# diff7/tts-king

Hardware: AMD Instinct MI355X
Metric: FS2 train mel-frames/sec/GPU + HiFi-GAN RTF (22.05 kHz), batch=16 (higher is better)
Workload: dtype bf16

## Files before the change

### include/ttsk.h

```cpp
#ifndef TTSK_H
#define TTSK_H

#include <stdint.h>

#ifdef __cplusplus
extern "C" {
#endif

#define TTSK_VERSION 1

#define TTSK_OK 0
#define TTSK_EINVAL (-1)
#define TTSK_ELAUNCH (-2)

int ttsk_version(void);
const char* ttsk_last_error(void);

enum {
  TTSK_GEMM_A_TR      = 1 << 0,
  TTSK_GEMM_B_TR      = 1 << 1,
  TTSK_GEMM_C_F32     = 1 << 2,
  TTSK_GEMM_RELU      = 1 << 3,
  TTSK_GEMM_ADD_R     = 1 << 4,
  TTSK_GEMM_R_F32     = 1 << 5,
  TTSK_GEMM_MASK_G    = 1 << 6,
  TTSK_GEMM_LRELU_IN  = 1 << 7,
  TTSK_GEMM_TANH      = 1 << 8,
  TTSK_GEMM_ACCUM_C   = 1 << 9,
  TTSK_GEMM_LRELU_OUT = 1 << 10,
  TTSK_GEMM_F16       = 1 << 11,
  TTSK_GEMM_C2_LRELU  = 1 << 12,
  TTSK_GEMM_DEFER_REDUCE = 1 << 13,
  TTSK_GEMM_RAW_SLABS = 1 << 14
};

typedef struct ttsk_gemm_desc {
  const void* A;
  const void* B;
  void* C;
  void* C2;
  const float* bias;
  const void* R;
  const void* G;
  int32_t M, N, K;
  int32_t lda, ldb, ldc, ldr, ldg;
  int32_t flags;
  float alpha;
  float in_slope, out_slope;
  int32_t nz1, nz2;
  int64_t sA1, sA2, sB1, sB2, sC1, sC2, sR1, sR2;
  int32_t taps, seg_len, tap_shift0, tap_dshift;
  int64_t b_tap_stride;
  int32_t bseg_len, bshift0, bdshift;
  int32_t out_seg, out_mul, out_add;
  int32_t out_add_dz;
  int32_t splits;
  void* workspace;
  int64_t workspace_bytes;
  int32_t kernel;
  int64_t s_bias1;
} ttsk_gemm_desc;

int ttsk_gemm(const ttsk_gemm_desc* d, void* stream);
typedef struct ttsk_reduce_item {
  const float* ws;
  float* C;
  int32_t M, N, ldc, nz, splits, accumulate;
  int64_t sC2;
  float alpha;
} ttsk_reduce_item;
int ttsk_gemm_reduce_batch(const ttsk_reduce_item* items, int n, void* stream);

int64_t ttsk_gemm_group_table_bytes(int n);
int ttsk_gemm_group_build(const ttsk_gemm_desc* descs, int n, void* host_table, int32_t* total_wgs);
int ttsk_gemm_group_launch(const void* host_table, void* dev_table, void* stream);
int ttsk_gemm_group_launch_capped(const void* host_table, void* dev_table, int max_wgs, void* stream);
int ttsk_gemm_group_upload(const void* host_table, void* dev_table, void* stream);
int ttsk_gemm_group_launch_uploaded(const void* host_table, void* dev_table, int max_wgs, void* stream);

int ttsk_ffn_conv_supported(int Cin, int Cout, int K);
int ttsk_ffn_conv_fwd(const void* x_bf16, const void* w_bf16, const float* bias, void* out_bf16, int B, int S, int Cin, int Cout, int K,
                      int relu, int packed, void* stream);
int ttsk_ffn_pack_weight(const void* w_bf16, void* packed_bf16, int Cout, int K, void* stream);
int ttsk_ffn_pack_weight_batch(const void* const* w_bf16, void* const* packed_bf16, int n , int Cout, int K, void* stream);
typedef struct ttsk_pack_item {
  const void* src;
  void* dst;
  int32_t Cs, K, Ds, transpose;
} ttsk_pack_item;
int ttsk_win_conv_supported(int Cin, int Cout, int K);
int ttsk_win_conv_pack_items(const ttsk_pack_item* items, int n, void* stream);
int ttsk_win_conv_pack_table(const ttsk_pack_item* dev_items, int n, void* stream);
int ttsk_win_conv_pack_batch(const void* const* w_bf16, void* const* packed_bf16, int n , int Cs, int K, int Ds, int transpose,
                             void* stream);
int ttsk_win_conv_split(const void* x_bf16, const void* w_packed, float* slabs, int nsplit, int B, int S, int Cin_total, int Cout, int K,
                        void* stream);
int ttsk_win_conv(const void* x_bf16, const void* w_packed, const float* bias , const void* gate_bf16 ,
                  const float* delta_o32 , float* delta_out , void* out, int out_f32, int B, int S, int Cin,
                  int Cout, int K, int relu, void* stream);
int ttsk_win_conv_stats_rows(int B, int S);
int ttsk_win_conv_resid(const void* x_bf16, const void* w_packed, const float* resid_f32, void* out_bf16, int B, int S, int Cin, int Cout,
                        int K, void* stream);
int ttsk_win_conv_dual(const void* x_bf16, const void* w_packed, const float* bias, float* out_f32, void* out_bf16, int B, int S, int Cin,
                       int Cout, int K, void* stream);
int ttsk_win_conv_stats(const void* x_bf16, const void* w_packed, const float* bias, float* out_f32, float* stats,
                        const int32_t* frame_limit, int B, int S, int Cin, int Cout, int K, void* stream);
int ttsk_win_conv_bnb(const void* x_bf16, const void* w_packed, void* out_bf16, float* stats, const float* bn_x_f32, const float* mean,
                      const float* rstd, const float* gamma, const float* beta, const uint8_t* keep, float p, int use_tanh,
                      const int32_t* frame_limit, int B, int S, int Cin, int Cout, int K, void* stream);
int ttsk_hifi_upsample8_supported(int Cin, int Cout);
int ttsk_hifi_upsample8(const void* x16, const void* w_packed, const float* bias8, void* out16, int f16, int B, int T, int Cin, int Cout,
                        void* stream);
int ttsk_hifi_upsample_win_supported(int Cin, int Cout, int stride);
int ttsk_hifi_upsample_win(const void* x16, const void* w_packed, const float* bias_rep, void* out16, int f16, int B, int T, int Cin, int Cout,
                           int stride, void* stream);
int ttsk_hifi_conv_pre_win_supported(int Cin, int Cout, int K);
int ttsk_hifi_conv_pre_win(const void* x16, const void* w_packed, const float* bias, void* out16, int f16, int B, int T, int Cin, int Cout, int K,
                           float slope, void* stream);
int ttsk_hifi_upsample_loop_supported(int Cin, int Cout, int stride);
int ttsk_hifi_upsample_loop(const void* x16, const void* w_packed, const float* bias_rep, void* out16, int f16, int B, int T, int Cin, int Cout,
                            int stride, void* stream);

int ttsk_gemm_ln_fwd(const void* A, int lda, const void* W, int ldw, const float* bias, const void* res, const float* gamma,
                     const float* beta, void* out, void* z_save, float* mean, float* rstd, const int64_t* lens, int seg_len,
                     int M, int K, int D, float eps, float p_pre, uint32_t site_pre, const void* rng, void* stream);
int ttsk_win_ln_supported(int K, int D);
int ttsk_win_ln_fwd(const void* A, int lda, const void* W_packed, const float* bias, const void* res, const float* gamma, const float* beta,
                    void* out, void* z_save, float* mean, float* rstd, const int64_t* lens, int seg_len, int M, int K, int D, float eps,
                    float p_pre, uint32_t site_pre, const void* rng, void* stream);
int ttsk_win_ln_proj_fwd(const void* A, int lda, const void* W_packed, const float* bias, const void* res, const float* gamma,
                         const float* beta, void* out, void* z_save, float* mean, float* rstd, const int64_t* lens, int seg_len, int M,
                         int K, int D, float eps, float p_pre, uint32_t site_pre, const void* rng, const void* proj_w_packed,
                         const float* proj_bias, int proj_Cout, void* proj_out, void* stream);

int ttsk_gemm_plan(const ttsk_gemm_desc* d, int32_t* kernel, int32_t* splits, int64_t* workspace_bytes);


int ttsk_length_regulator_fwd(const void* x_bf16, const void* dur, int dur_dtype, const float* pe, void* out_bf16,
                              int32_t* idx_out ,
                              int32_t* cumsum_out , int64_t* mel_len , int B, int L, int T, int D,
                              void* stream);
int ttsk_length_regulator_bwd(const void* dout_bf16, const int32_t* cumsum, void* dx_bf16, int B, int L, int T, int D,
                              void* stream);

int ttsk_layernorm_fwd(const void* y_bf16, const void* res_bf16, const float* gamma, const float* beta, void* out_bf16,
                       void* z_save_bf16, float* mean, float* rstd, const int64_t* lens, int seg_len, int rows, int D,
                       float eps, float p_pre, uint32_t site_pre, float p_post, uint32_t site_post, const uint64_t* rng,
                       const float* head_w, const float* head_b, float* head_out, void* stream);
int ttsk_layernorm_bwd_nblocks(int rows);
int ttsk_layernorm_bwd(const void* dout_bf16, const float* dhead, const float* head_w, const void* z_bf16, const float* mean,
                       const float* rstd, const float* gamma, const float* beta, const int64_t* lens, int seg_len, int rows,
                       int D, int relu_in, float p_pre, uint32_t site_pre, float p_post, uint32_t site_post,
                       const uint64_t* rng, void* dz_bf16, void* dy_bf16, float* partials, void* stream);
int ttsk_layernorm_fwd_grouped(const void* y_bf16, const void* res_bf16, const float* gamma, const float* beta, void* out_bf16,
                               void* z_save_bf16, float* mean, float* rstd, const int64_t* lens, int seg_len, int groups,
                               int group_rows, int64_t param_stride, uint32_t site_stride, int D, float eps, float p_pre,
                               uint32_t site_pre, float p_post, uint32_t site_post, const uint64_t* rng, const float* head_w,
                               const float* head_b, float* head_out, void* stream);
int ttsk_layernorm_bwd_grouped(const void* dout_bf16, const float* dhead, const float* head_w, const void* z_bf16,
                               const float* mean, const float* rstd, const float* gamma, const float* beta, const int64_t* lens,
                               int seg_len, int groups, int group_rows, int64_t param_stride, uint32_t site_stride, int D,
                               int relu_in, float p_pre, uint32_t site_pre, float p_post, uint32_t site_post, const uint64_t* rng,
                               void* dz_bf16, void* dy_bf16, float* partials, void* stream);
int ttsk_layernorm_bwd_slabs(const float* slabs, int nsplit, int64_t slab_stride, const void* R_bf16, const void* z_bf16,
                             const float* mean, const float* rstd, const float* gamma, const float* beta, const int64_t* lens,
                             int seg_len, int rows, int D, int relu_in, float p_pre, uint32_t site_pre, float p_post,
                             uint32_t site_post, const uint64_t* rng, void* dz_bf16, void* dy_bf16, float* partials, void* stream);
int ttsk_layernorm_bwd_proj_nblocks(int rows);
int ttsk_layernorm_bwd_proj(const void* dout_bf16, const float* slabs, int nsplit, int64_t slab_stride, const void* R_bf16,
                            const void* z_bf16, const float* mean, const float* rstd, const float* gamma, const int64_t* lens,
                            int seg_len, int rows, int D, float p_pre, uint32_t site_pre, const uint64_t* rng, void* dz_bf16,
                            void* dy_bf16, float* partials, const void* w_packed, int Cout, const void* gate_bf16,
                            const float* delta_o32, float* delta_out, void* out_bf16, const void* pre_x_bf16,
                            const void* pre_w_packed, int pre_K, void* stream);
int ttsk_qkv_dx(const void* dqkv_bf16, const void* w_packed, const void* R_bf16, void* out_bf16, int rows, int K, int D, void* stream);
int ttsk_colsum_finalize(const float* partials, int nblk, int ncols, int ld, float* dst, int accumulate, float scale,
                         void* stream);
typedef struct ttsk_finalize_item {
  const float* partials;
  float* dst;
  int32_t nblk, ncols, ld, accumulate;
  float scale;
} ttsk_finalize_item;
int ttsk_colsum_finalize_batch(const ttsk_finalize_item* items, int n, void* stream);
int ttsk_colsum_nblocks(int rows);
int ttsk_colsum(const void* x, int is_f32, int rows, int C, int ld, float* partials, void* stream);
typedef struct ttsk_colsum_item {
  const void* x;
  float* partials;
  int32_t is_f32, rows, C, ld, nblk;
} ttsk_colsum_item;
int ttsk_colsum_batch(const ttsk_colsum_item* items, int n, void* stream);

int ttsk_va_embed(const void* x_bf16, const float* speaker_table, const int64_t* speakers, int L, const float* pitch_target,
                  const float* pitch_bins, const float* pitch_table, const float* energy_target, const float* energy_bins,
                  const float* energy_table, int n_bins_minus_1, void* x1_bf16, void* x2_bf16, void* x3_bf16, int32_t* pitch_idx,
                  int32_t* energy_idx, int rows, int D, const int64_t* row_limit, void* stream);
int ttsk_va_combine(const void* dx3_bf16, const float* dxin, void* dx2_bf16, void* dx1_bf16, void* dx_bf16, int rows, int D, int L,
                    const int64_t* row_limit, void* stream);

int ttsk_softmax_fwd(const float* scores, void* probs_bf16, const int64_t* lens, int nz, int H, int S, int Sp, void* stream);
int ttsk_softmax_bwd(const void* probs_bf16, const float* dprobs, void* dscores_bf16, int nz, int S, int Sp, float alpha,
                     void* stream);

int ttsk_flash_attention_fwd(const void* qkv_bf16, void* o_bf16, float* o_f32 , float* lse ,
                             const int64_t* lens, int B, int H, int S, int d, float scale, void* stream);
int ttsk_flash_attention_bwd(const void* qkv_bf16, const void* o_bf16, const float* o_f32 , const void* dout_bf16,
                             const float* lse, float* delta_ws, int delta_ready, void* dqkv_bf16, const int64_t* lens, int B, int H, int S,
                             int d, float scale, void* stream);

int ttsk_bucketize(const float* values, const float* bins, int n_bins, float scale, int32_t* idx, float* scaled_out,
                   int n, void* stream);
int ttsk_duration_round(const float* logd, float d_control, float* out, int n, void* stream);
int ttsk_length_mask(const int64_t* lens, uint8_t* mask, int B, int T, void* stream);
int ttsk_add_f32(const float* a, const float* b, float scale_b, float* out, int64_t n, void* stream);
int ttsk_gather_add(const void* in_bf16, const float* table, const void* idx, int idx_is_i64, int idx_div, const float* pe,
                    int pe_mod, void* out_bf16, int rows, int D, void* stream);
int ttsk_scatter_sum(const void* dx_bf16, const void* idx, int idx_is_i64, int idx_div, int n_idx, float* dtable,
                     int n_table_rows, int D, int skip_row, int accumulate, void* stream);
int ttsk_gather_add_lens(const void* in_bf16, const float* table, const int64_t* idx, const int64_t* lens, int seg_len,
                         void* out_bf16, int rows, int D, void* stream);
int ttsk_embed_step(const float* pred, const float* control, const float* bins, int n_bins, const float* table,
                    const void* x_bf16, const int64_t* lens, int seg_len, void* x_out_bf16, float* scaled_out,
                    int32_t* idx_out, int rows, int D, void* stream);
int ttsk_duration_round_dev(const float* logd, const float* d_control, int L, float* out, int n, void* stream);
int ttsk_embed_step_rows(const float* pred, const float* control, const float* value, const uint8_t* has, const float* bins,
                         int n_bins, const float* table, const void* x_bf16, const int64_t* lens, int seg_len, void* x_out_bf16,
                         float* scaled_out, int32_t* idx_out, int rows, int D, void* stream);
int ttsk_duration_rows(const float* logd, const float* d_control, const float* durations, const uint8_t* has, float* out, int n,
                       void* stream);
int ttsk_duration_fit(const float* v, const uint8_t* has, const int32_t* target, const int64_t* lens, int seg_len, float* out,
                      int B, void* stream);
typedef struct ttsk_scatter_item {
  const void* dx;
  const void* idx;
  float* dtable;
  int32_t idx_is_i64, idx_div, n_idx, n_table_rows, D, skip_row, accumulate;
} ttsk_scatter_item;
int ttsk_scatter_sum_batch(const ttsk_scatter_item* items, int n, void* stream);

int ttsk_cast_bf16(const float* src, void* dst_bf16, int64_t n, void* stream);
int ttsk_nct_to_ntc(const float* src, void* dst16, int f16, int B, int C, int T, void* stream);
int ttsk_to_int16(const float* src, int16_t* dst, int64_t n, float scale, void* stream);

#define TTSK_WIN_ROW 8
#define TTSK_WIN_VALID 6
int ttsk_mel_windows(const float* src, int64_t stride_t, int64_t stride_c, int64_t n_src_frames, const int32_t* plan, void* dst16,
                     int f16, int N, int W, int C, void* stream);
int ttsk_wav_stitch(const float* src, const int32_t* plan, void* dst, int64_t n_dst_frames, int to_i16, float scale, int N, int W,
                    int spf, void* stream);

int ttsk_weight_norm_fold(const float* v, const float* g, float* w, int rows, int cols, void* stream);
int ttsk_pack_conv_weight(const float* src, void* dst16, int f16, int d0, int d1, int d2, int mode, void* stream);
int ttsk_hifi_conv_window_supported(int C, int K, int dil);
int ttsk_hifi_conv_window(const void* x16, const void* w_pack, const float* bias, const void* R16, void* out16, void* out2_16,
                          int f16, int B, int len, int C, int K, int dil, int lrelu_out, float slope, void* stream);
int ttsk_hifi_conv_pair_supported(int C, int K, int dil);
int ttsk_hifi_conv_pair(const void* x16, const void* w1_pack, const float* bias1, const void* w2_pack, const float* bias2, void* out16,
                        int f16, int B, int len, int C, int K, int dil, float slope, int mode, float scale, float final_slope,
                        void* stream);
int ttsk_hifi_conv_pair_ws_supported(int C, int K, int dil);
int ttsk_hifi_conv_pair_ws(const void* x16, const void* w1_pack, const float* bias1, const void* w2_pack, const float* bias2, void* out16,
                           int f16, int B, int len, int C, int K, int dil, float slope, int mode, float scale, float final_slope,
                           int max_wgs, void* stream);
int ttsk_hifi_resblock2_supported(int C, int K, int d0, int d1);
int ttsk_hifi_resblock2(const void* x16, const void* w0_pack, const float* bias0, const void* w1_pack, const float* bias1, void* out16,
                        int f16, int B, int len, int C, int K, int d0, int d1, float slope, int mode, float scale, float final_slope,
                        void* stream);
int ttsk_hifi_conv_post(const void* x16, const void* w16, const float* bias, float* out, int f16, int B, int len, int C, int K,
                        void* stream);
int ttsk_hifi_upsample2_supported(int Cin, int Cout, int stride, int k);
int ttsk_hifi_upsample2(const void* x16, const void* w16, const float* bias, void* out16, int f16, int B, int T, int Cin,
                        int Cout, void* stream);
int ttsk_avg3(const void* a, const void* b, const void* c, void* out, int f16, int64_t n, float scale, float slope, void* stream);

int64_t ttsk_resblock_pack_elems(int C, int K);
int ttsk_pack_resblock_weight(const float* src, void* dst16, int f16, int C, int K, void* stream);
int ttsk_hifi_resblock1(const void* x16, void* out16, int f16, const void* const* weights, const float* const* biases,
                        const int32_t* dilations, int B, int len, int C, int K, int mode, float scale, float slope,
                        float final_slope, void* stream);
int ttsk_hifi_resblock1_supported(int C, int K);
int ttsk_hifi_mrf32_post_supported(int C, int k0, int k1, int k2, int k_post);
int ttsk_hifi_mrf32_post(const void* x16, float* out, void* stage_out16, int f16, const void* const* weights, const float* const* biases,
                         const int32_t* dilations, const void* w_post16, const float* b_post, int B, int len, int C, int k0, int k1, int k2,
                         int k_post, float slope, float final_slope, float scale, void* stream);

int ttsk_hifi_conv_pair_rowlen(const void* x16, const void* w1_pack, const float* bias1, const void* w2_pack, const float* bias2, void* out16,
                             int f16, int B, int len, int C, int K, int dil, float slope, int mode, float scale, float final_slope,
                             const int32_t* row_frames, int row_stride, int spf, void* stream);
int ttsk_hifi_conv_pair_ws_rowlen(const void* x16, const void* w1_pack, const float* bias1, const void* w2_pack, const float* bias2,
                                void* out16, int f16, int B, int len, int C, int K, int dil, float slope, int mode, float scale,
                                float final_slope, int max_wgs, const int32_t* row_frames, int row_stride, int spf, void* stream);
int ttsk_hifi_resblock2_rowlen(const void* x16, const void* w0_pack, const float* bias0, const void* w1_pack, const float* bias1, void* out16,
                             int f16, int B, int len, int C, int K, int d0, int d1, float slope, int mode, float scale, float final_slope,
                             const int32_t* row_frames, int row_stride, int spf, void* stream);
int ttsk_hifi_resblock1_rowlen(const void* x16, void* out16, int f16, const void* const* weights, const float* const* biases,
                             const int32_t* dilations, int B, int len, int C, int K, int mode, float scale, float slope,
                             float final_slope, const int32_t* row_frames, int row_stride, int spf, void* stream);
int ttsk_hifi_mrf32_post_rowlen(const void* x16, float* out, void* stage_out16, int f16, const void* const* weights,
                              const float* const* biases, const int32_t* dilations, const void* w_post16, const float* b_post, int B,
                              int len, int C, int k0, int k1, int k2, int k_post, float slope, float final_slope, float scale,
                              const int32_t* row_frames, int row_stride, int spf, void* stream);
int ttsk_zero_rows_past(void* x16, int B, int len, int C, const int32_t* row_frames, int row_stride, int spf, void* stream);

int ttsk_zero_frames_from(void* x, int elem_bytes, int rows, int C, int seg_len, const int32_t* frame_limit, void* stream);

int ttsk_zero_frames_lens(void* x, int elem_bytes, int rows, int C, int seg_len, const int64_t* lens, void* stream);

int ttsk_bn_nblocks(int rows);
int ttsk_bn_stats(const void* x, int x_is_f32, int rows, int C, float* partials , const int32_t* frame_limit,
                  int seg_len, void* stream);
int ttsk_bn_finalize(const float* partials, int nblk, int C, int rows, float eps, float momentum, float* mean, float* rstd,
                     float* running_mean, float* running_var, int64_t* num_batches_tracked, const int32_t* frame_limit, int seg_len,
                     void* stream);
int ttsk_rsqrt_eps(const float* var, float eps, float* rstd, int n, void* stream);
int ttsk_bn_nchunks(int rows);
int ttsk_bn_stats_slab(const void* x, int x_is_f32, int rows, int C, float* partials , const int32_t* frame_limit,
                       int seg_len, void* stream);
int ttsk_bn_train_apply(const void* x, int x_is_f32, const float* partials, int nblk, float eps, float momentum, float* mean,
                        float* rstd, float* running_mean, float* running_var, int64_t* num_batches_tracked, const float* gamma,
                        const float* beta, int rows, int C, int use_tanh, float p, uint32_t site, const uint64_t* rng,
                        const float* resid_f32, void* out_bf16, float* out_f32, uint8_t* keep_out, const int32_t* frame_limit,
                        int seg_len, void* stream);
int ttsk_bn_bwd_stats_slab(const void* dout, int dout_is_f32, const void* x, int x_is_f32, const float* mean, const float* rstd,
                           const float* gamma, const float* beta, int rows, int C, int use_tanh, float p, uint32_t site,
                           const uint64_t* rng, const uint8_t* keep, float* partials ,
                           const int32_t* frame_limit, int seg_len, void* stream);
int ttsk_bn_bwd_apply_slab(const void* dout, int dout_is_f32, const void* x, int x_is_f32, const float* mean, const float* rstd,
                           const float* gamma, const float* beta, int rows, int C, int use_tanh, float p, uint32_t site,
                           const uint64_t* rng, const uint8_t* keep, const float* partials, int nblk, void* dx_bf16, float* dgamma,
                           float* dbeta, int accumulate , const int32_t* frame_limit, int seg_len,
                           void* stream);
int ttsk_bn_apply(const void* x, int x_is_f32, const float* mean, const float* rstd, const float* gamma, const float* beta, int rows,
                  int C, int use_tanh, float p, uint32_t site, const uint64_t* rng, const float* resid_f32, void* out_bf16,
                  float* out_f32, const int32_t* frame_limit, int seg_len, void* stream);
int ttsk_bn_apply_lens(const void* x, int x_is_f32, const float* mean, const float* rstd, const float* gamma, const float* beta,
                       int rows, int C, int use_tanh, const float* resid_f32, void* out_bf16, float* out_f32, const int64_t* lens,
                       int seg_len, void* stream);
int ttsk_bn_bwd_stats(const void* dout, int dout_is_f32, const void* x, int x_is_f32, const float* mean, const float* rstd,
                      const float* gamma, const float* beta, int rows, int C, int use_tanh, float p, uint32_t site,
                      const uint64_t* rng, float* partials , const int32_t* frame_limit,
                      int seg_len, void* stream);
int ttsk_bn_bwd_apply(const void* dout, int dout_is_f32, const void* x, int x_is_f32, const float* mean, const float* rstd,
                      const float* gamma, const float* beta, int rows, int C, int use_tanh, float p, uint32_t site,
                      const uint64_t* rng, const float* sums , void* dx_bf16, float* dgamma, float* dbeta,
                      int accumulate , const int32_t* frame_limit, int seg_len, void* stream);

int ttsk_fs2_loss_nblocks(void);
int ttsk_fs2_loss(const float* mel, const float* post, const float* mel_target, const int64_t* mel_lens, const float* pitch,
                  const float* energy, const float* logd, const float* pitch_target, const float* energy_target,
                  const int64_t* dur_target, const int64_t* src_lens, int B, int T, int T_target, int n_mel, int L,
                  float grad_scale, float* dmel_sum, float* dpost, float* dpitch, float* denergy, float* dlogd,
                  float* partials, float* losses, const int32_t* frame_limit, void* stream);
int ttsk_fs2_loss_mel(const float* mel, const float* post, const float* mel_target, const int64_t* mel_lens, int B, int T, int T_target,
                      int n_mel, float grad_scale, float* dmel_sum, float* dpost, float* partials, const int32_t* frame_limit, void* stream);
int ttsk_fs2_loss_var(const float* pitch, const float* energy, const float* logd, const float* pitch_target, const float* energy_target,
                      const int64_t* dur_target, const int64_t* src_lens, int B, int L, float grad_scale, float* dpitch, float* denergy,
                      float* dlogd, float* partials, void* stream);
int ttsk_fs2_loss_finalize(const float* partials_mel, const float* partials_var, const int64_t* src_lens, int B, int T, int n_mel,
                           const int32_t* frame_limit, float* losses, void* stream);

int ttsk_optim_state_bytes(void);
int ttsk_optim_advance(void* state, float d_model, float warmup, const float* anneal_steps_host, int n_anneal,
                       float anneal_rate, float beta1, float beta2, void* stream);
int ttsk_rng_advance(void* state, void* stream);
int ttsk_dropout_keep_mask(const uint64_t* rng, uint32_t site, int64_t n, float p, uint8_t* keep, void* stream);
int ttsk_clip_adam_step(float* params, float* grads, float* exp_avg, float* exp_avg_sq, void* shadow_bf16, int64_t n,
                        void* state, float* partials, float max_norm, float beta1, float beta2, float eps, int zero_grad,
                        void* stream);
int ttsk_grad_sumsq(const float* grads, int64_t n, float* partials, void* stream);
int ttsk_optim_step(float* params, float* grads, float* exp_avg, float* exp_avg_sq, void* shadow_bf16, int64_t n, void* state,
                    float* partials, float max_norm, float beta1, float beta2, float eps, int zero_grad, float d_model, float warmup,
                    const float* anneal_steps_host, int n_anneal, float anneal_rate, int advance_rng, void* stream);

typedef struct ttsk_dwconv_item {
  const void* dy;
  const void* x;
  float* dw;
  const int64_t* lens;
  int32_t Cout, Cin, K, ldy, ldx, B, S, accumulate;
} ttsk_dwconv_item;
int ttsk_dwconv_supported(int Cout, int Cin, int K);
int ttsk_dwconv_batch(const ttsk_dwconv_item* items, int n , void* stream);

typedef struct ttsk_dwgemm_item {
  const void* dy;
  const void* x;
  float* dw;
  float* workspace;
  const int64_t* lens;
  int32_t Cout, Cin, K, ldy, ldx, B, S, accumulate, splits;
} ttsk_dwgemm_item;
int ttsk_dwgemm_supported(int Cout, int Cin, int K);
int64_t ttsk_dwgemm_workspace_floats(int Cout, int Cin, int K, int splits);
int ttsk_dwgemm_batch(const ttsk_dwgemm_item* items, int n , int max_wgs, void* stream);

typedef struct ttsk_adam_item {
  int64_t off;
  void* pack;
  void* pack_t;
  int32_t Cs, K, Ds, tile0;
} ttsk_adam_item;
int ttsk_optim_step_packed(float* params, float* grads, float* exp_avg, float* exp_avg_sq, void* shadow_bf16, int64_t n, void* state,
                           float* partials, float max_norm, float beta1, float beta2, float eps, int zero_grad, float d_model, float warmup,
                           const float* anneal_steps_host, int n_anneal, float anneal_rate, int advance_rng,
                           const ttsk_adam_item* dev_items, int n_items, int n_tiles, const int64_t* dev_gaps, int n_gaps,
                           int64_t gap_floats, void* stream);
int ttsk_optim_step_ranges(float* params, float* grads, float* exp_avg, float* exp_avg_sq, void* shadow_bf16, int64_t n, void* state,
                           float* partials, float max_norm, float beta1, float beta2, float eps, int zero_grad, float d_model, float warmup,
                           const float* anneal_steps_host, int n_anneal, float anneal_rate, int advance_rng,
                           const int64_t* dev_ranges, int n_ranges, int64_t range_floats,
                           const ttsk_adam_item* dev_items, int n_items, int n_tiles, const int64_t* dev_gaps, int n_gaps,
                           int64_t gap_floats, void* stream);

#define TTSK_CWT_CHANNELS 11
#define TTSK_CNNSCALAR_BINS 30
#define TTSK_CNNSCALAR_FLOATS 456
int ttsk_layernorm_head_bwd_nblocks(int rows);
int ttsk_layernorm_head_fwd(const void* y_bf16, const float* gamma, const float* beta, const int64_t* lens, int seg_len, int rows, int D,
                            int n_out, float eps, float p_post, uint32_t site_post, const uint64_t* rng, const float* head_w,
                            const float* head_b, float* mean, float* rstd, float* head_out, void* stream);
int ttsk_layernorm_head_bwd(const float* dhead, const float* head_w, const void* z_bf16, const float* mean, const float* rstd,
                            const float* gamma, const float* beta, const int64_t* lens, int seg_len, int rows, int D, int n_out,
                            float p_post, uint32_t site_post, const uint64_t* rng, void* dz_bf16, float* partials, void* stream);
int ttsk_cnnscalar_fwd(const void* x_bf16, const float* cwt, const float* params, int B, int L, int D, float* rowdot, float* pooled,
                       float* stats, float* pre, float* out, void* stream);
int ttsk_cnnscalar_bwd(const float* dout, const void* x_bf16, const float* cwt, const float* params, const float* pooled,
                       const float* stats, const float* pre, int B, int L, int D, float* rowdot, float* partials, void* stream);
int ttsk_cwt_pitch(const float* cwt, const float* heads, const float* bins, int n_bins, float p_control, int B, int L, float* pitch,
                   int32_t* idx, void* stream);
int ttsk_fs2_loss_cwt(const float* cwt, const float* cwt_target, const float* heads, const float* mean_target, const float* std_target,
                      const int64_t* src_lens, int B, int L, float grad_scale, float* dcwt, float* dheads, float* losses, void* stream);

int ttsk_stft_frames(const float* wav, void* out16, int B, int len, int pad, int rows, int hop, float scale, void* stream);
int ttsk_mel_from_spec(const float* spec, int ld, const float* basis_vals, const int32_t* basis_start,
                       const int32_t* basis_off, int nnz, float* mel, float* energy, int B, int rows, int T, int nbins,
                       int n_mels, float eps, float clip, void* stream);

#ifdef __cplusplus
}
#endif
#endif
```

### tts_king_amd/csrc/dwgemm.hip

```cpp
#include "gemm_common.h"

namespace {

constexpr int DWG_NW = 8, DWG_NT = DWG_NW * 64, DWG_MAXP = 28, DWG_OOB = 0x7FFFFFFF;
constexpr int DWG_BK = 32, DWG_IMG = 1024 + 32;
constexpr int DWG_OPND = 16 * DWG_IMG;
constexpr int DWG_STAGE = 2 * DWG_OPND, DWG_NSTAGE = 3;
constexpr int DWG_SMEM = DWG_NSTAGE * DWG_STAGE;

struct DwgProblem {
  const bf16_t* dy;
  const bf16_t* x;
  float* out;
  const long long* lens;
  int Cout, Cin, taps, ldy, ldx, B, S, accumulate, splits;
  int wg0, nwg, tiles_m, tiles_n;
};
struct DwgArgs {
  DwgProblem p[DWG_MAXP];
  int n;
};

__device__ __forceinline__ void dwgemm_tile(const DwgArgs& args, int id, unsigned char* smem) {
  const int tid = threadIdx.x, lane = tid & 63, wave = tid >> 6;
  const int l15 = lane & 15, lg = lane >> 4;
  const int wm = wave >> 1, wn = wave & 1;
  int pi = 0;
  for (int i = 1; i < args.n; ++i)
    if (id >= args.p[i].wg0) pi = i;
  pi = __builtin_amdgcn_readfirstlane(pi);
  const DwgProblem& P = args.p[pi];
  int local = id - P.wg0;
  const int tile_n = local % P.tiles_n; local /= P.tiles_n;
  const int tap = local % P.taps; local /= P.taps;
  const int tile_m = local % P.tiles_m;
  const int split = local / P.tiles_m;
  const int m0 = tile_m * 256, n0 = tile_n * 256;
  const int S = P.S, ldy = P.ldy, ldx = P.ldx;
  const int shift = tap - P.taps / 2;
  const int b0 = (int)((long long)split * P.B / P.splits), b1 = (int)((long long)(split + 1) * P.B / P.splits);
  const int nB = b1 - b0;

  int nb_lane = 0;
  if (lane < nB) {
    nb_lane = S;
    if (P.lens) { const long long v = P.lens[b0 + lane]; nb_lane = v < 0 ? 0 : (v > S ? S : (int)v); }
  }
  int nsteps = 0;
  for (int b = 0; b < nB; ++b) nsteps += (__builtin_amdgcn_readlane(nb_lane, b) + DWG_BK - 1) / DWG_BK;

  const __amdgpu_buffer_rsrc_t rsA = __builtin_amdgcn_make_buffer_rsrc((void*)P.dy, 0, 0x7FFFFFF0, 0x00020000);
  const __amdgpu_buffer_rsrc_t rsB = __builtin_amdgcn_make_buffer_rsrc((void*)P.x, 0, 0x7FFFFFF0, 0x00020000);

  const int f_row = lane >> 5, f_c = lane & 31;
  const int f_lds = (f_c >> 1) * DWG_IMG + f_row * 32 + (f_c & 1) * 16;
  const int a_col = (m0 + f_c * 8) * 2, b_col = (n0 + f_c * 8) * 2;
  int ib = 0, ij = 0, inb = 0, loaded = 0;
  while (ib < nB && (inb = __builtin_amdgcn_readlane(nb_lane, ib)) == 0) ++ib;
  typedef __attribute__((ext_vector_type(4))) unsigned u32x4;
  auto load_piece = [&](int q, bool live) __attribute__((always_inline)) -> u32x4 {
    const int p = 2 * wave + (q & 1);
    const int row = ij * DWG_BK + 2 * p + f_row;
    if (q < 2) {
      const int off = ((b0 + ib) * S + row) * ldy * 2 + a_col;
      const bool ok = live & (row < inb);
      return __builtin_amdgcn_raw_buffer_load_b128(rsA, ok ? off : DWG_OOB, 0, 0);
    } else {
      const int t = row + shift;
      const int off = ((b0 + ib) * S + t) * ldx * 2 + b_col;
      const bool ok = live & (row < inb) & (t >= 0) & (t < S);
      return __builtin_amdgcn_raw_buffer_load_b128(rsB, ok ? off : DWG_OOB, 0, 0);
    }
  };
  auto load_advance = [&]() __attribute__((always_inline)) {
    ++loaded;
    if (++ij * DWG_BK >= inb) {
      ij = 0;
      ++ib;
      while (ib < nB && (inb = __builtin_amdgcn_readlane(nb_lane, ib)) == 0) ++ib;
    }
  };
  auto store_piece = [&](unsigned char* stage, int q, u32x4 v) __attribute__((always_inline)) {
    const int p = 2 * wave + (q & 1);
    *(u32x4*)(stage + (q < 2 ? 0 : DWG_OPND) + f_lds + p * 64) = v;
  };

  f32x4 acc[4][8];
#pragma unroll
  for (int i = 0; i < 4; ++i)
#pragma unroll
    for (int j = 0; j < 8; ++j) acc[i][j] = f32x4{0.f, 0.f, 0.f, 0.f};

  const int r0 = 16 * (lg >> 1) + 4 * (lg & 1) + (l15 >> 2), cq = (l15 & 3) << 3;
  const int a_lane = (wm * 4) * DWG_IMG + r0 * 32 + cq;
  const int b_lane = DWG_OPND + (wn * 8) * DWG_IMG + r0 * 32 + cq;
  typedef __attribute__((address_space(3))) bf16x4* tr_ptr;
  auto read_a = [&](const unsigned char* st, int i) __attribute__((always_inline)) -> bf16x8 {
    bf16x4 lo = __builtin_amdgcn_ds_read_tr16_b64_v4i16((tr_ptr)(st + a_lane + i * DWG_IMG));
    bf16x4 hi = __builtin_amdgcn_ds_read_tr16_b64_v4i16((tr_ptr)(st + a_lane + i * DWG_IMG + 256));
    return bf16x8{lo[0], lo[1], lo[2], lo[3], hi[0], hi[1], hi[2], hi[3]};
  };
  auto read_b = [&](const unsigned char* st, int j) __attribute__((always_inline)) -> bf16x8 {
    bf16x4 lo = __builtin_amdgcn_ds_read_tr16_b64_v4i16((tr_ptr)(st + b_lane + j * DWG_IMG));
    bf16x4 hi = __builtin_amdgcn_ds_read_tr16_b64_v4i16((tr_ptr)(st + b_lane + j * DWG_IMG + 256));
    return bf16x8{lo[0], lo[1], lo[2], lo[3], hi[0], hi[1], hi[2], hi[3]};
  };

#define DWG_SB() __builtin_amdgcn_sched_barrier(0)
#define DWG_BARRIER() asm volatile("s_barrier" ::: "memory")
  if (nsteps > 0) {
    u32x4 set[2][4];
    const int nsteps2 = (nsteps + 1) & ~1;
#pragma unroll
    for (int n = 0; n < 2; ++n) {
#pragma unroll
      for (int q = 0; q < 4; ++q) set[n][q] = load_piece(q, loaded < nsteps);
      if (loaded < nsteps) load_advance();
    }
#pragma unroll
    for (int n = 0; n < 2; ++n) {
#pragma unroll
      for (int q = 0; q < 4; ++q) store_piece(smem + n * DWG_STAGE, q, set[n][q]);
      const bool more = loaded < nsteps;
#pragma unroll
      for (int q = 0; q < 4; ++q) set[n][q] = load_piece(q, more);
      if (more) load_advance();
    }
    asm volatile("s_waitcnt lgkmcnt(0)" ::: "memory");
    DWG_BARRIER();
    const unsigned char* st = smem;
    unsigned char* stw = smem + 2 * DWG_STAGE;
    bf16x8 af[2][4], bf[3];
#pragma unroll
    for (int i = 0; i < 4; ++i) af[0][i] = read_a(st, i);
    bf[0] = read_b(st, 0);
    bf[1] = read_b(st, 1);
    auto do_step = [&](int par, bf16x8 (&ac)[4], bf16x8 (&an)[4]) __attribute__((always_inline)) {
      const bool more = loaded < nsteps;
      const unsigned char* stn = (st == smem + 2 * DWG_STAGE) ? smem : st + DWG_STAGE;
      DWG_SB();
#pragma unroll
      for (int j = 0; j < 8; ++j) {
        if (j + 2 < 8) bf[(j + 2) % 3] = read_b(st, j + 2);
        if ((j & 1) == 0) {
          const int q = j >> 1;
          store_piece(stw, q, set[par][q]);
          set[par][q] = load_piece(q, more);
          if (q == 3 && more) load_advance();
        }
        if (j >= 2 && j < 6) an[j - 2] = read_a(stn, j - 2);
        if (j >= 6) bf[(j + 2) % 3] = read_b(stn, j + 2 - 8);
#pragma unroll
        for (int i = 0; i < 4; ++i) acc[i][j] = mfma16<false>(ac[i], bf[j % 3], acc[i][j]);
        DWG_SB();
      }
      DWG_BARRIER();
      st = stn;
      stw = (stw == smem + 2 * DWG_STAGE) ? smem : stw + DWG_STAGE;
    };
#pragma unroll 1
    for (int step = 0; step < nsteps2; step += 2) {
      do_step(0, af[0], af[1]);
      { const bf16x8 t0 = bf[2], t1 = bf[0]; bf[0] = t0; bf[1] = t1; }
      do_step(1, af[1], af[0]);
      { const bf16x8 t0 = bf[2], t1 = bf[0]; bf[0] = t0; bf[1] = t1; }
    }
  }
#undef DWG_SB
#undef DWG_BARRIER

  const int Cin = P.Cin, Cout = P.Cout, taps = P.taps;
  const bool slab = P.splits > 1;
  float* base = slab ? P.out + ((int64_t)(split * taps + tap) * Cout) * Cin : P.out + (int64_t)tap * Cin;
  const int64_t rstride = slab ? (int64_t)Cin : (int64_t)taps * Cin;
  const bool accumulate = !slab && P.accumulate;
#pragma unroll
  for (int i = 0; i < 4; ++i) {
#pragma unroll
    for (int r = 0; r < 4; ++r) {
      float* row = base + (int64_t)(m0 + wm * 64 + i * 16 + 4 * lg + r) * rstride + n0 + wn * 128 + l15;
      if (accumulate) {
        float old[8];
#pragma unroll
        for (int j = 0; j < 8; ++j) old[j] = row[j * 16];
#pragma unroll
        for (int j = 0; j < 8; ++j) row[j * 16] = old[j] + acc[i][j][r];
      } else {
#pragma unroll
        for (int j = 0; j < 8; ++j) row[j * 16] = acc[i][j][r];
      }
    }
  }
}

__global__ __launch_bounds__(DWG_NT, 1) void dwgemm_kernel(const DwgArgs args, int total) {
  __shared__ __attribute__((aligned(16))) unsigned char smem[DWG_SMEM];
  for (int w = blockIdx.x; w < total; w += gridDim.x) {
    const int q = total >> 3, r = total & 7, x = w & 7;
    const int id = (x < r ? x * (q + 1) : r * (q + 1) + (x - r) * q) + (w >> 3);
    dwgemm_tile(args, id, smem);
    __syncthreads();
  }
}

}

extern "C" int ttsk_dwgemm_supported(int Cout, int Cin, int K) {
  return K >= 1 && K <= 15 && (K & 1) == 1 && Cout > 0 && Cin > 0 && Cout % 256 == 0 && Cin % 256 == 0;
}

extern "C" int64_t ttsk_dwgemm_workspace_floats(int Cout, int Cin, int K, int splits) {
  return splits > 1 ? (int64_t)splits * K * Cout * Cin : 0;
}

extern "C" int ttsk_dwgemm_batch(const ttsk_dwgemm_item* items, int n, int max_wgs, void* stream) {
  TTSK_REQUIRE(items && n > 0 && n <= DWG_MAXP, "dwgemm_batch: 1..%d items", DWG_MAXP);
  DwgArgs a;
  a.n = n;
  int wg = 0;
  for (int i = 0; i < n; ++i) {
    const ttsk_dwgemm_item& it = items[i];
    TTSK_REQUIRE(it.dy && it.x && it.dw, "dwgemm_batch: null pointer in item %d", i);
    TTSK_REQUIRE(ttsk_dwgemm_supported(it.Cout, it.Cin, it.K), "dwgemm_batch: no instance for Cout=%d Cin=%d K=%d", it.Cout, it.Cin, it.K);
    TTSK_REQUIRE(it.B > 0 && it.S > 0 && it.splits >= 1 && it.splits <= it.B && (it.B + it.splits - 1) / it.splits <= 64,
                 "dwgemm_batch: B=%d utterances in %d splits (at most 64 per split)", it.B, it.splits);
    TTSK_REQUIRE(it.splits == 1 || it.workspace, "dwgemm_batch: splits > 1 needs a workspace of ttsk_dwgemm_workspace_floats");
    TTSK_REQUIRE(it.ldy >= it.Cout && it.ldx >= it.Cin && (it.ldy & 7) == 0 && (it.ldx & 7) == 0, "dwgemm_batch: row pitches (multiples of 8, >= channels)");
    TTSK_REQUIRE((int64_t)it.B * it.S * (it.ldy > it.ldx ? it.ldy : it.ldx) * 2 < 0x7FFFFFF0ll, "dwgemm_batch: operand beyond the 2 GiB buffer range");
    TTSK_REQUIRE(((((uintptr_t)it.dy) | ((uintptr_t)it.x) | ((uintptr_t)it.dw) | ((uintptr_t)it.workspace)) & 15) == 0, "dwgemm_batch: 16-byte alignment");
    DwgProblem& p = a.p[i];
    p.dy = (const bf16_t*)it.dy; p.x = (const bf16_t*)it.x; p.lens = (const long long*)it.lens;
    p.out = it.splits > 1 ? it.workspace : it.dw;
    p.Cout = it.Cout; p.Cin = it.Cin; p.taps = it.K; p.ldy = it.ldy; p.ldx = it.ldx; p.B = it.B; p.S = it.S;
    p.accumulate = it.accumulate; p.splits = it.splits;
    p.tiles_m = it.Cout / 256; p.tiles_n = it.Cin / 256;
    p.nwg = p.tiles_m * p.tiles_n * it.K * it.splits;
    p.wg0 = wg;
    wg += p.nwg;
  }
  TTSK_REQUIRE(max_wgs >= 0, "dwgemm_batch: max_wgs >= 0 (0 = a workgroup per tile)");
  hipLaunchKernelGGL(dwgemm_kernel, dim3(max_wgs > 0 && max_wgs < wg ? max_wgs : wg), dim3(DWG_NT), 0, (hipStream_t)stream, a, wg);
  TTSK_CHECK_LAUNCH();
  return TTSK_OK;
}
```

Baseline: 2.461 million.

## Split dwgemm tiles into sub-tile parts when tiles underfill the chip

When the weight-gradient GEMM has few 256x256 tiles relative to the compute-unit count, each tile is split into 2, 4 or 8 smaller parts (128x256, 128x128, 64x128) and launched on a leaner kernel with smaller shared memory. This raises the number of workgroups so more CUs take part. A new schedule also splits the leftover tail wave of a persistent grid into parts and alternates XCD order across slots. The cost is lower per-workgroup reuse, more redundant operand loads, and extra template instances.

```diff
diff --git a/include/ttsk.h b/include/ttsk.h
--- a/include/ttsk.h
+++ b/include/ttsk.h
@@ -394,6 +394,8 @@
 int ttsk_dwgemm_supported(int Cout, int Cin, int K);
 int64_t ttsk_dwgemm_workspace_floats(int Cout, int Cin, int K, int splits);
 int ttsk_dwgemm_batch(const ttsk_dwgemm_item* items, int n , int max_wgs, void* stream);
+int ttsk_dwgemm_grid(int total, int max_wgs, int cus);
+int ttsk_dwgemm_schedule(int total, int grid, int32_t* units);
 
 typedef struct ttsk_adam_item {
   int64_t off;
diff --git a/tts_king_amd/csrc/dwgemm.hip b/tts_king_amd/csrc/dwgemm.hip
--- a/tts_king_amd/csrc/dwgemm.hip
+++ b/tts_king_amd/csrc/dwgemm.hip
@@ -1,4 +1,5 @@
 #include "gemm_common.h"
+#include "dwgemm_schedule.h"
 
 namespace {
 
@@ -21,7 +22,10 @@
   int n;
 };
 
-__device__ __forceinline__ void dwgemm_tile(const DwgArgs& args, int id, unsigned char* smem) {
+template <int PARTS, bool LEAN = false>
+__device__ __forceinline__ void dwgemm_tile(const DwgArgs& args, int id, int part, unsigned char* smem) {
+  constexpr int TM = dwg_part_rows(PARTS), TN = dwg_part_cols(PARTS), MI = TM / 64, NJ = TN / 32;
+  constexpr int OPND = LEAN ? (TM / 16) * DWG_IMG : DWG_OPND, STAGE = LEAN ? ((TM + TN) / 16) * DWG_IMG : DWG_STAGE;
   const int tid = threadIdx.x, lane = tid & 63, wave = tid >> 6;
   const int l15 = lane & 15, lg = lane >> 4;
   const int wm = wave >> 1, wn = wave & 1;
@@ -35,7 +39,7 @@
   const int tap = local % P.taps; local /= P.taps;
   const int tile_m = local % P.tiles_m;
   const int split = local / P.tiles_m;
-  const int m0 = tile_m * 256, n0 = tile_n * 256;
+  const int m0 = tile_m * 256 + dwg_part_row0(PARTS, part), n0 = tile_n * 256 + dwg_part_col0(PARTS, part);
   const int S = P.S, ldy = P.ldy, ldx = P.ldx;
   const int shift = tap - P.taps / 2;
   const int b0 = (int)((long long)split * P.B / P.splits), b1 = (int)((long long)(split + 1) * P.B / P.splits);
@@ -52,20 +56,27 @@
   const __amdgpu_buffer_rsrc_t rsA = __builtin_amdgcn_make_buffer_rsrc((void*)P.dy, 0, 0x7FFFFFF0, 0x00020000);
   const __amdgpu_buffer_rsrc_t rsB = __builtin_amdgcn_make_buffer_rsrc((void*)P.x, 0, 0x7FFFFFF0, 0x00020000);
 
-  const int f_row = lane >> 5, f_c = lane & 31;
-  const int f_lds = (f_c >> 1) * DWG_IMG + f_row * 32 + (f_c & 1) * 16;
-  const int a_col = (m0 + f_c * 8) * 2, b_col = (n0 + f_c * 8) * 2;
+  constexpr int LA = TM / 8, LB = TN / 8;
+  constexpr int RA = 64 / LA, RB = 64 / LB;
+  constexpr int NPA = 32 / RA, NPB = 32 / RB;
+  constexpr int QA = NPA >= 8 ? NPA / 8 : 1, QB = NPB / 8, NQ = QA + QB;
+  static_assert(2 * NQ <= NJ && NQ <= 4, "a piece is stored every other fragment column of a K step");
+  const int fa_row = lane / LA, fa_c = lane % LA, fb_row = lane / LB, fb_c = lane % LB;
+  const int fa_lds = (fa_c >> 1) * DWG_IMG + fa_row * 32 + (fa_c & 1) * 16;
+  const int fb_lds = (fb_c >> 1) * DWG_IMG + fb_row * 32 + (fb_c & 1) * 16;
+  const int a_col = (m0 + fa_c * 8) * 2, b_col = (n0 + fb_c * 8) * 2;
+  const bool a_mine = NPA >= 8 || wave < NPA;
   int ib = 0, ij = 0, inb = 0, loaded = 0;
   while (ib < nB && (inb = __builtin_amdgcn_readlane(nb_lane, ib)) == 0) ++ib;
   typedef __attribute__((ext_vector_type(4))) unsigned u32x4;
   auto load_piece = [&](int q, bool live) __attribute__((always_inline)) -> u32x4 {
-    const int p = 2 * wave + (q & 1);
-    const int row = ij * DWG_BK + 2 * p + f_row;
-    if (q < 2) {
+    if (q < QA) {
+      const int row = ij * DWG_BK + RA * (QA * wave + q) + fa_row;
       const int off = ((b0 + ib) * S + row) * ldy * 2 + a_col;
-      const bool ok = live & (row < inb);
+      const bool ok = live & a_mine & (row < inb);
       return __builtin_amdgcn_raw_buffer_load_b128(rsA, ok ? off : DWG_OOB, 0, 0);
     } else {
+      const int row = ij * DWG_BK + RB * (QB * wave + q - QA) + fb_row;
       const int t = row + shift;
       const int off = ((b0 + ib) * S + t) * ldx * 2 + b_col;
       const bool ok = live & (row < inb) & (t >= 0) & (t < S);
@@ -81,19 +92,22 @@
     }
   };
   auto store_piece = [&](unsigned char* stage, int q, u32x4 v) __attribute__((always_inline)) {
-    const int p = 2 * wave + (q & 1);
-    *(u32x4*)(stage + (q < 2 ? 0 : DWG_OPND) + f_lds + p * 64) = v;
-  };
-
-  f32x4 acc[4][8];
-#pragma unroll
-  for (int i = 0; i < 4; ++i)
-#pragma unroll
-    for (int j = 0; j < 8; ++j) acc[i][j] = f32x4{0.f, 0.f, 0.f, 0.f};
+    if (q < QA) {
+      if (a_mine) *(u32x4*)(stage + fa_lds + (QA * wave + q) * (RA * 32)) = v;
+    } else {
+      *(u32x4*)(stage + OPND + fb_lds + (QB * wave + q - QA) * (RB * 32)) = v;
+    }
+  };
+
+  f32x4 acc[MI][NJ];
+#pragma unroll
+  for (int i = 0; i < MI; ++i)
+#pragma unroll
+    for (int j = 0; j < NJ; ++j) acc[i][j] = f32x4{0.f, 0.f, 0.f, 0.f};
 
   const int r0 = 16 * (lg >> 1) + 4 * (lg & 1) + (l15 >> 2), cq = (l15 & 3) << 3;
-  const int a_lane = (wm * 4) * DWG_IMG + r0 * 32 + cq;
-  const int b_lane = DWG_OPND + (wn * 8) * DWG_IMG + r0 * 32 + cq;
+  const int a_lane = (wm * MI) * DWG_IMG + r0 * 32 + cq;
+  const int b_lane = OPND + (wn * NJ) * DWG_IMG + r0 * 32 + cq;
   typedef __attribute__((address_space(3))) bf16x4* tr_ptr;
   auto read_a = [&](const unsigned char* st, int i) __attribute__((always_inline)) -> bf16x8 {
     bf16x4 lo = __builtin_amdgcn_ds_read_tr16_b64_v4i16((tr_ptr)(st + a_lane + i * DWG_IMG));
@@ -109,61 +123,62 @@
 #define DWG_SB() __builtin_amdgcn_sched_barrier(0)
 #define DWG_BARRIER() asm volatile("s_barrier" ::: "memory")
   if (nsteps > 0) {
-    u32x4 set[2][4];
+    u32x4 set[2][NQ];
     const int nsteps2 = (nsteps + 1) & ~1;
 #pragma unroll
     for (int n = 0; n < 2; ++n) {
 #pragma unroll
-      for (int q = 0; q < 4; ++q) set[n][q] = load_piece(q, loaded < nsteps);
+      for (int q = 0; q < NQ; ++q) set[n][q] = load_piece(q, loaded < nsteps);
       if (loaded < nsteps) load_advance();
     }
 #pragma unroll
     for (int n = 0; n < 2; ++n) {
 #pragma unroll
-      for (int q = 0; q < 4; ++q) store_piece(smem + n * DWG_STAGE, q, set[n][q]);
+      for (int q = 0; q < NQ; ++q) store_piece(smem + n * STAGE, q, set[n][q]);
       const bool more = loaded < nsteps;
 #pragma unroll
-      for (int q = 0; q < 4; ++q) set[n][q] = load_piece(q, more);
+      for (int q = 0; q < NQ; ++q) set[n][q] = load_piece(q, more);
       if (more) load_advance();
     }
     asm volatile("s_waitcnt lgkmcnt(0)" ::: "memory");
     DWG_BARRIER();
     const unsigned char* st = smem;
-    unsigned char* stw = smem + 2 * DWG_STAGE;
-    bf16x8 af[2][4], bf[3];
-#pragma unroll
-    for (int i = 0; i < 4; ++i) af[0][i] = read_a(st, i);
+    unsigned char* stw = smem + 2 * STAGE;
+    bf16x8 af[2][MI], bf[3];
+#pragma unroll
+    for (int i = 0; i < MI; ++i) af[0][i] = read_a(st, i);
     bf[0] = read_b(st, 0);
     bf[1] = read_b(st, 1);
-    auto do_step = [&](int par, bf16x8 (&ac)[4], bf16x8 (&an)[4]) __attribute__((always_inline)) {
+    constexpr int A0 = NJ - MI >= 2 ? 2 : 0;
+    auto do_step = [&](int par, bf16x8 (&ac)[MI], bf16x8 (&an)[MI]) __attribute__((always_inline)) {
       const bool more = loaded < nsteps;
-      const unsigned char* stn = (st == smem + 2 * DWG_STAGE) ? smem : st + DWG_STAGE;
+      const unsigned char* stn = (st == smem + 2 * STAGE) ? smem : st + STAGE;
       DWG_SB();
 #pragma unroll
-      for (int j = 0; j < 8; ++j) {
-        if (j + 2 < 8) bf[(j + 2) % 3] = read_b(st, j + 2);
-        if ((j & 1) == 0) {
+      for (int j = 0; j < NJ; ++j) {
+        if (j + 2 < NJ) bf[(j + 2) % 3] = read_b(st, j + 2);
+        if ((j & 1) == 0 && (j >> 1) < NQ) {
           const int q = j >> 1;
           store_piece(stw, q, set[par][q]);
           set[par][q] = load_piece(q, more);
-          if (q == 3 && more) load_advance();
+          if (q == NQ - 1 && more) load_advance();
         }
-        if (j >= 2 && j < 6) an[j - 2] = read_a(stn, j - 2);
-        if (j >= 6) bf[(j + 2) % 3] = read_b(stn, j + 2 - 8);
-#pragma unroll
-        for (int i = 0; i < 4; ++i) acc[i][j] = mfma16<false>(ac[i], bf[j % 3], acc[i][j]);
+        if (j >= A0 && j < A0 + MI) an[j - A0] = read_a(stn, j - A0);
+        if (j + 2 >= NJ) bf[(j + 2) % 3] = read_b(stn, j + 2 - NJ);
+#pragma unroll
+        for (int i = 0; i < MI; ++i) acc[i][j] = mfma16<false>(ac[i], bf[j % 3], acc[i][j]);
         DWG_SB();
       }
       DWG_BARRIER();
       st = stn;
-      stw = (stw == smem + 2 * DWG_STAGE) ? smem : stw + DWG_STAGE;
+      stw = (stw == smem + 2 * STAGE) ? smem : stw + STAGE;
     };
 #pragma unroll 1
     for (int step = 0; step < nsteps2; step += 2) {
       do_step(0, af[0], af[1]);
-      { const bf16x8 t0 = bf[2], t1 = bf[0]; bf[0] = t0; bf[1] = t1; }
+      { const bf16x8 t0 = bf[NJ % 3], t1 = bf[(NJ + 1) % 3]; bf[0] = t0; bf[1] = t1; }
       do_step(1, af[1], af[0]);
-      { const bf16x8 t0 = bf[2], t1 = bf[0]; bf[0] = t0; bf[1] = t1; }
+      { const bf16x8 t0 = bf[NJ % 3], t1 = bf[(NJ + 1) % 3]; bf[0] = t0; bf[1] = t1; }
     }
   }
 #undef DWG_SB
@@ -175,19 +190,19 @@
   const int64_t rstride = slab ? (int64_t)Cin : (int64_t)taps * Cin;
   const bool accumulate = !slab && P.accumulate;
 #pragma unroll
-  for (int i = 0; i < 4; ++i) {
+  for (int i = 0; i < MI; ++i) {
 #pragma unroll
     for (int r = 0; r < 4; ++r) {
-      float* row = base + (int64_t)(m0 + wm * 64 + i * 16 + 4 * lg + r) * rstride + n0 + wn * 128 + l15;
+      float* row = base + (int64_t)(m0 + wm * (16 * MI) + i * 16 + 4 * lg + r) * rstride + n0 + wn * (16 * NJ) + l15;
       if (accumulate) {
-        float old[8];
-#pragma unroll
-        for (int j = 0; j < 8; ++j) old[j] = row[j * 16];
-#pragma unroll
-        for (int j = 0; j < 8; ++j) row[j * 16] = old[j] + acc[i][j][r];
+        float old[NJ];
+#pragma unroll
+        for (int j = 0; j < NJ; ++j) old[j] = row[j * 16];
+#pragma unroll
+        for (int j = 0; j < NJ; ++j) row[j * 16] = old[j] + acc[i][j][r];
       } else {
 #pragma unroll
-        for (int j = 0; j < 8; ++j) row[j * 16] = acc[i][j][r];
+        for (int j = 0; j < NJ; ++j) row[j * 16] = acc[i][j][r];
       }
     }
   }
@@ -195,14 +210,50 @@
 
 __global__ __launch_bounds__(DWG_NT, 1) void dwgemm_kernel(const DwgArgs args, int total) {
   __shared__ __attribute__((aligned(16))) unsigned char smem[DWG_SMEM];
-  for (int w = blockIdx.x; w < total; w += gridDim.x) {
-    const int q = total >> 3, r = total & 7, x = w & 7;
-    const int id = (x < r ? x * (q + 1) : r * (q + 1) + (x - r) * q) + (w >> 3);
-    dwgemm_tile(args, id, smem);
+  const int slots = total / (int)gridDim.x + 1;
+  for (int s = 0; s < slots; ++s) {
+    const DwgUnit u = dwg_schedule(total, gridDim.x, blockIdx.x, s);
+    if (u.tile < 0) break;
+    switch (u.parts) {
+      case 1: dwgemm_tile<1>(args, u.tile, 0, smem); break;
+      case 2: dwgemm_tile<2>(args, u.tile, u.part, smem); break;
+      case 4: dwgemm_tile<4>(args, u.tile, u.part, smem); break;
+      default: dwgemm_tile<8>(args, u.tile, u.part, smem); break;
+    }
     __syncthreads();
   }
 }
 
+int dwg_device_cus() {
+  static int cus[64] = {};
+  int dev = 0, v = 0;
+  if (hipGetDevice(&dev) != hipSuccess || dev < 0 || dev >= 64) return -1;
+  if (cus[dev] > 0) return cus[dev];
+  if (hipDeviceGetAttribute(&v, hipDeviceAttributeMultiprocessorCount, dev) != hipSuccess || v <= 0) return -1;
+  return cus[dev] = v;
+}
+
+template <int PARTS>
+__global__ __launch_bounds__(DWG_NT) void dwgemm_parts_kernel(const DwgArgs args, int total) {
+  __shared__ __attribute__((aligned(16))) unsigned char smem[DWG_NSTAGE * ((dwg_part_rows(PARTS) + dwg_part_cols(PARTS)) / 16) * DWG_IMG];
+  const DwgUnit u = dwg_schedule(total, gridDim.x, blockIdx.x, 0);
+  if (u.tile >= 0) dwgemm_tile<PARTS, true>(args, u.tile, u.part, smem);
+}
+
+}
+
+extern "C" int ttsk_dwgemm_grid(int total, int max_wgs, int cus) { return dwg_grid(total, max_wgs, cus); }
+
+extern "C" int ttsk_dwgemm_schedule(int total, int grid, int32_t* units) {
+  TTSK_REQUIRE(units && total > 0 && grid > 0, "dwgemm_schedule: total, grid > 0 and a table of (total / grid + 1) * grid * 7 ints");
+  for (int s = 0; s <= total / grid; ++s)
+    for (int w = 0; w < grid; ++w) {
+      const DwgUnit u = dwg_schedule(total, grid, w, s);
+      int32_t* o = units + ((int64_t)s * grid + w) * 7;
+      o[0] = u.tile; o[1] = u.part; o[2] = u.parts;
+      o[3] = dwg_part_row0(u.parts, u.part); o[4] = dwg_part_col0(u.parts, u.part); o[5] = dwg_part_rows(u.parts); o[6] = dwg_part_cols(u.parts);
+    }
+  return TTSK_OK;
 }
 
 extern "C" int ttsk_dwgemm_supported(int Cout, int Cin, int K) {
@@ -238,8 +289,18 @@
     p.wg0 = wg;
     wg += p.nwg;
   }
-  TTSK_REQUIRE(max_wgs >= 0, "dwgemm_batch: max_wgs >= 0 (0 = a workgroup per tile)");
-  hipLaunchKernelGGL(dwgemm_kernel, dim3(max_wgs > 0 && max_wgs < wg ? max_wgs : wg), dim3(DWG_NT), 0, (hipStream_t)stream, a, wg);
+  TTSK_REQUIRE(max_wgs >= 0, "dwgemm_batch: max_wgs >= 0 (0 = a workgroup per tile, or per part of one when the tiles fill at most half the chip)");
+  int cus = 0;
+  if (max_wgs == 0) {
+    cus = dwg_device_cus();
+    TTSK_REQUIRE(cus > 0, "dwgemm_batch: cannot read the device's compute-unit count");
+  }
+  const int grid = dwg_grid(wg, max_wgs, cus);
+  const int parts = grid > wg ? dwg_parts(wg, grid) : 1;
+  if (parts == 8) hipLaunchKernelGGL(dwgemm_parts_kernel<8>, dim3(grid), dim3(DWG_NT), 0, (hipStream_t)stream, a, wg);
+  else if (parts == 4) hipLaunchKernelGGL(dwgemm_parts_kernel<4>, dim3(grid), dim3(DWG_NT), 0, (hipStream_t)stream, a, wg);
+  else if (parts == 2) hipLaunchKernelGGL(dwgemm_parts_kernel<2>, dim3(grid), dim3(DWG_NT), 0, (hipStream_t)stream, a, wg);
+  else hipLaunchKernelGGL(dwgemm_kernel, dim3(grid), dim3(DWG_NT), 0, (hipStream_t)stream, a, wg);
   TTSK_CHECK_LAUNCH();
   return TTSK_OK;
 }
diff --git a/tts_king_amd/csrc/dwgemm_schedule.h b/tts_king_amd/csrc/dwgemm_schedule.h
--- /dev/null
+++ b/tts_king_amd/csrc/dwgemm_schedule.h
@@ -0,0 +1,48 @@
+#pragma once
+
+#if defined(__HIPCC__)
+#define DWG_HD __host__ __device__ inline
+#else
+#define DWG_HD inline
+#endif
+
+struct DwgUnit {
+  int tile, part, parts;
+};
+
+DWG_HD constexpr int dwg_part_rows(int P) { return P == 1 ? 256 : P <= 4 ? 128 : 64; }
+DWG_HD constexpr int dwg_part_cols(int P) { return P <= 2 ? 256 : 128; }
+DWG_HD constexpr int dwg_part_row0(int P, int part) { return (P <= 2 ? part : part >> 1) * dwg_part_rows(P); }
+DWG_HD constexpr int dwg_part_col0(int P, int part) { return P <= 2 ? 0 : (part & 1) * 128; }
+
+DWG_HD int dwg_xcd_major(int total, int u) {
+  const int q = total >> 3, r = total & 7, x = u & 7;
+  return (x < r ? x * (q + 1) : r * (q + 1) + (x - r) * q) + (u >> 3);
+}
+
+DWG_HD int dwg_parts(int rem, int G) { return rem <= G / 8 ? 8 : rem <= G / 4 ? 4 : rem <= G / 2 ? 2 : 1; }
+
+DWG_HD DwgUnit dwg_schedule(int total, int G, int w, int s) {
+  const DwgUnit none = {-1, 0, 1};
+  const int R = total / G, rem = total - R * G;
+  if (s < R) return DwgUnit{s * G + dwg_xcd_major(G, (s & 1) && (G & 7) == 0 ? w ^ 7 : w), 0, 1};
+  if (s > R || rem == 0) return none;
+  const int P = dwg_parts(rem, G);
+  int v, part;
+  if (((rem + 7) >> 3) * 8 * P <= G) {
+    const int k = w >> 3;
+    v = (k / P) * 8 + (w & 7);
+    part = k % P;
+  } else {
+    v = w / P;
+    part = w % P;
+  }
+  if (v >= rem) return none;
+  return DwgUnit{(R & 1) ? total - 1 - dwg_xcd_major(rem, v) : R * G + dwg_xcd_major(rem, v), part, P};
+}
+
+DWG_HD int dwg_grid(int total, int max_wgs, int cus) {
+  if (max_wgs > 0 && max_wgs < total) return max_wgs;
+  if (max_wgs == 0 && total > 0 && total <= cus / 2) return total * dwg_parts(total, cus);
+  return total;
+}
```

Result: no change. 2.453 million (-0.4%).
